# cocowy1/PPMStereo

Hardware: AMD Instinct MI355X
Metric: disparity-px/s (higher is better)
Workload: dtype bf16; 1 GPU; BASELINE config 2: T=5 clip at 320x512, iters=10, hot path only (3-scale cascade from encoder outputs: corr pyramid build + lookup, QAM pick, pick-and-play memory attention, ConvGRU3D update, heads, convex upsample, test_mode=True as PPMStereo.forward_batch_test calls it: predictions[-1] is the output, so the mask head, the convex upsampling and the full-resolution resize run only where their resu; T=5, H=320, W=512, iters=10, parallelism=replicas x1

## Files before the change

### include/ppms.h

```cpp
#ifndef PPMS_H
#define PPMS_H
#include <stdint.h>

#ifdef __cplusplus
extern "C" {
#endif

#define PPMS_OK 0
#define PPMS_EINVAL (-1)
#define PPMS_ELAUNCH (-2)
#define PPMS_ENODEV (-3)

#define PPMS_ABI_VERSION 4

int ppms_version(void);
const char* ppms_last_error(void);
int ppms_device_info(char* name, int name_cap, int* cu_count, int* clock_mhz);

int ppms_corr_build(const float* fmap1, const float* fmap2, float* const pyr[5], int B, int C, int H, int W, void* stream);

int ppms_corr_lookup(const float* const pyr[4], const float* flow, int flow_nhwc, float* out_nchw, void* out_hi, void* out_lo,
                     int out_ld, void* flow_sp_hi, void* flow_sp_lo, int flow_sp_ld, int B, int H, int W, void* stream);

typedef struct ppms_sp {
// ... 43 lines not shown
    ppms_epilogue epi[2];
} ppms_conv;

int ppms_conv_gemm2(const ppms_conv* desc, const ppms_conv* dev_desc, int wm_hint, void* stream);
int ppms_conv_gemm2_slices(const ppms_conv* desc);
int64_t ppms_conv_gemm2_slice_workspace_bytes(const ppms_conv* desc, int nslice);
int ppms_conv_gemm2_sliced(const ppms_conv* desc, const ppms_conv* dev_desc, int nslice, void* workspace, void* stream);
int ppms_conv_gemm2_ysweep_slices(const ppms_conv* desc);
int ppms_conv_gemm2_ysweep(const ppms_conv* desc, const ppms_conv* dev_desc, int nslice, void* workspace, void* stream);
int ppms_conv_gemm5_applicable(const ppms_conv* desc);
int ppms_conv_gemm5(const ppms_conv* desc, const ppms_conv* dev_desc, int nbt, void* stream);
int ppms_conv_gemm5_slices(const ppms_conv* desc);
int ppms_conv_gemm5_sliced(const ppms_conv* desc, const ppms_conv* dev_desc, int nbt, int nslice, void* workspace, void* stream);
int ppms_conv_gemm6_applicable(const ppms_conv* desc);
int ppms_conv_gemm6(const ppms_conv* desc, const ppms_conv* dev_desc, void* stream);
int ppms_gemm1_applicable(const ppms_conv* desc);
int ppms_gemm1(const ppms_conv* desc, const ppms_conv* dev_desc, int cb_hint, void* stream);
int ppms_conv_stream_applicable(const ppms_conv* desc);
int ppms_conv_stream(const ppms_conv* desc, const ppms_conv* dev_desc, int hint, void* stream);
int ppms_struct_sizes(int* sp, int* epilogue, int* conv);

int ppms_dwconv_gelu(ppms_sp x, ppms_sp y, const float* w, const float* b, int k, int BT, int H, int W, void* stream);
int ppms_flow_patch7(const float* flow_nhwc, ppms_sp patch, int BT, int H, int W, void* stream);
int ppms_unc_tail(ppms_sp x, const float* w, float bias, float* unc, float* partial, int BT, int HW, void* stream);

int ppms_nchw_to_sp(const float* src, ppms_sp dst, int BT, int C, int HW, void* stream);
int ppms_sp_to_nchw(ppms_sp src, float* dst, int BT, int C, int HW, void* stream);
int ppms_nchw_to_nhwc(const float* src, float* dst, int dst_ld, int BT, int C, int HW, void* stream);
int ppms_nhwc_to_nchw(const float* src, int src_ld, float* dst, int BT, int C, int HW, void* stream);
int ppms_f32_to_sp(const float* src, int src_ld, ppms_sp dst, int64_t pixels, void* stream);
// ... 103 lines not shown
```

### ppmstereo_amd/_lib.py

```python
from __future__ import annotations

import ctypes as C
import os
from typing import Optional

import torch

from . import build as _build

c_void_p, c_int, c_float, c_int64 = C.c_void_p, C.c_int, C.c_float, C.c_int64

EPI_STORE, EPI_RESID, EPI_RH, EPI_GRU, EPI_ADDF32 = range(5)
ATTN_P_BF16, ATTN_P_FP16 = 0, 1
ACT_NONE, ACT_RELU, ACT_GELU, ACT_SIGMOID, ACT_TANH, ACT_ELU1 = range(6)


def vt_image(v: torch.Tensor, p_format: int) -> torch.Tensor:
    b = v.to(torch.bfloat16)
    if p_format == ATTN_P_BF16:
        return b.contiguous()
    return b.float().clamp(-65504.0, 65504.0).to(torch.float16).contiguous().view(torch.bfloat16)


def vt_values(vt: torch.Tensor, p_format: int) -> torch.Tensor:
# ... 4 lines not shown
    _fields_ = [("hi", c_void_p), ("lo", c_void_p), ("ld", C.c_int32), ("c", C.c_int32)]


class Epilogue(C.Structure):
    _fields_ = [("kind", C.c_int32), ("act", C.c_int32), ("scale", c_float), ("n_valid", C.c_int32),
                ("out_sp", SP), ("out_f32", c_void_p), ("out_f32_ld", C.c_int32), ("vt_f16", C.c_int32), ("out_vt", c_void_p),
                ("aux_sp", SP), ("aux_f32", c_void_p), ("aux_f32_ld", C.c_int32), ("pre_f32_ld", C.c_int32),
                ("pre_f32", c_void_p)]


class Conv(C.Structure):
    _fields_ = [("seg", SP * 2), ("nseg", C.c_int32), ("groups", C.c_int32), ("w", c_void_p), ("bias", c_void_p),
                ("T", C.c_int32), ("H", C.c_int32), ("W", C.c_int32),
                ("kt", C.c_int32), ("kh", C.c_int32), ("kw", C.c_int32),
                ("M", C.c_int32), ("m_split", C.c_int32), ("t_halo", C.c_int32), ("lo_zero_from", C.c_int32), ("epi", Epilogue * 2)]


class ChainLayer(C.Structure):
    _fields_ = [("w", c_void_p), ("bias", c_void_p), ("post_s", c_void_p), ("post_t", c_void_p),
                ("M", C.c_int32), ("n_valid", C.c_int32), ("resid", C.c_int32)]


class ChainParams(C.Structure):
    _fields_ = [("inp", SP), ("out", SP), ("layer", ChainLayer * 3), ("nlayers", C.c_int32), ("P", C.c_int64)]


class YUVView(C.Structure):
    _fields_ = [("y", c_void_p), ("u", c_void_p), ("v", c_void_p), ("frame_stride_y", c_int64), ("frame_stride_c", c_int64),
                ("pitch_y", C.c_int32), ("pitch_c", C.c_int32), ("step_c", C.c_int32), ("reserved", C.c_int32)]

# ... 29 lines not shown
                                 c_int, c_int, c_int, c_int, c_void_p]),
    "ppms_conv_gemm2": (c_int, [C.POINTER(Conv), c_void_p, c_int, c_void_p]),
    "ppms_conv_gemm2_slices": (c_int, [C.POINTER(Conv)]),
    "ppms_conv_gemm2_slice_workspace_bytes": (C.c_int64, [C.POINTER(Conv), c_int]),
    "ppms_conv_gemm2_sliced": (c_int, [C.POINTER(Conv), c_void_p, c_int, c_void_p, c_void_p]),
    "ppms_conv_gemm2_ysweep_slices": (c_int, [C.POINTER(Conv)]),
    "ppms_conv_gemm2_ysweep": (c_int, [C.POINTER(Conv), c_void_p, c_int, c_void_p, c_void_p]),
    "ppms_gemm1_applicable": (c_int, [C.POINTER(Conv)]),
    "ppms_gemm1": (c_int, [C.POINTER(Conv), c_void_p, c_int, c_void_p]),
    "ppms_conv_stream_applicable": (c_int, [C.POINTER(Conv)]),
    "ppms_conv_stream": (c_int, [C.POINTER(Conv), c_void_p, c_int, c_void_p]),
    "ppms_conv_gemm5_applicable": (c_int, [C.POINTER(Conv)]),
    "ppms_conv_gemm5": (c_int, [C.POINTER(Conv), c_void_p, c_int, c_void_p]),
    "ppms_conv_gemm6_applicable": (c_int, [C.POINTER(Conv)]),
    "ppms_conv_gemm6": (c_int, [C.POINTER(Conv), c_void_p, c_void_p]),
    "ppms_conv_gemm5_slices": (c_int, [C.POINTER(Conv)]),
    "ppms_conv_gemm5_sliced": (c_int, [C.POINTER(Conv), c_void_p, c_int, c_int, c_void_p, c_void_p]),
    "ppms_struct_sizes": (c_int, [C.POINTER(c_int), C.POINTER(c_int), C.POINTER(c_int)]),
    "ppms_dwconv_gelu": (c_int, [SP, SP, c_void_p, c_void_p, c_int, c_int, c_int, c_int, c_void_p]),
    "ppms_flow_patch7": (c_int, [c_void_p, SP, c_int, c_int, c_int, c_void_p]),
    "ppms_unc_tail": (c_int, [SP, c_void_p, c_float, c_void_p, c_void_p, c_int, c_int, c_void_p]),
    "ppms_nchw_to_sp": (c_int, [c_void_p, SP, c_int, c_int, c_int, c_void_p]),
    "ppms_sp_to_nchw": (c_int, [SP, c_void_p, c_int, c_int, c_int, c_void_p]),
    "ppms_nchw_to_nhwc": (c_int, [c_void_p, c_void_p, c_int, c_int, c_int, c_int, c_void_p]),
    "ppms_nhwc_to_nchw": (c_int, [c_void_p, c_int, c_void_p, c_int, c_int, c_int, c_void_p]),
    "ppms_f32_to_sp": (c_int, [c_void_p, c_int, SP, c_int64, c_void_p]),
    "ppms_sp_to_f32": (c_int, [SP, c_void_p, c_int, c_int64, c_void_p]),
    "ppms_tap_gather_sum": (c_int, [c_void_p, c_int, c_void_p, c_void_p, c_int, c_void_p, c_int, c_int, c_int, c_int, c_int, c_int, c_int, c_int, c_int, c_void_p]),
    "ppms_flow_add": (c_int, [c_void_p, c_void_p, c_int, c_int64, c_void_p]),
    "ppms_convex_upsample": (c_int, [c_void_p, c_void_p, c_int, c_void_p, c_int, c_int, c_int, c_void_p]),
# ... 57 lines not shown
    try:
        path = _build.build(verbose=not os.path.exists(_build.LIB))
        lib = C.CDLL(path)
    except Exception as exc:
        raise RuntimeError(f"ppmstereo_amd: the HIP library libppms.so is missing and could not be built ({exc}); "
                           "there is no CPU fallback") from exc
    for name, (res, args) in _SIGS.items():
        fn = getattr(lib, name)
        fn.restype, fn.argtypes = res, args
    if lib.ppms_version() != 4:
        raise RuntimeError("ppmstereo_amd: libppms.so ABI version mismatch")
    a, b, c = c_int(), c_int(), c_int()
    lib.ppms_struct_sizes(C.byref(a), C.byref(b), C.byref(c))
    if (a.value, b.value, c.value) != (C.sizeof(SP), C.sizeof(Epilogue), C.sizeof(Conv)):
        raise RuntimeError("ppmstereo_amd: ctypes struct layout differs from include/ppms.h")
    lib.ppms_yuv_struct_sizes(C.byref(a), C.byref(b))
    if (a.value, b.value) != (C.sizeof(YUVView), C.sizeof(YUVMatrix)):
        raise RuntimeError("ppmstereo_amd: ctypes layout of ppms_yuv_view / ppms_yuv_matrix differs from include/ppms.h")
    lib.ppms_remap_struct_size(C.byref(a))
    if a.value != C.sizeof(RemapView):
        raise RuntimeError("ppmstereo_amd: ctypes layout of ppms_remap_view differs from include/ppms.h")
    if lib.ppms_egress_struct_size() != C.sizeof(Egress):
        raise RuntimeError("ppmstereo_amd: ctypes layout of ppms_egress differs from include/ppms.h")
    if lib.ppms_pwchain_param_bytes() != C.sizeof(ChainParams):
        raise RuntimeError("ppmstereo_amd: ChainParams layout differs from pwchain.hip")
    _lib = lib
    return lib


def check(rc: int) -> None:
# ... 48 lines not shown
```

### ppmstereo_amd/convplan.py

```python
from __future__ import annotations

import ctypes as C
from typing import Dict, Optional, Sequence

import torch

from . import _lib as L
from . import packing as _packing

CONV2 = 2
CONV5 = 5
GEMM1 = 6
STREAM = 7
CONV6 = 8
CONV2_SWEPT = "2s"
KERNEL_NAMES = {CONV2: "conv_gemm2", CONV5: "conv_gemm5", GEMM1: "gemm1", STREAM: "conv_stream", CONV6: "conv_gemm6"}
ALL_KERNELS = frozenset((CONV2, CONV2_SWEPT, CONV5, GEMM1, STREAM, CONV6))

TUNING = dict(
    conv6_grouped=True,
    attn_p="fp16",
)

KERNEL_TIMING = {"on": True}


def attn_p_format() -> int:
    fmt = TUNING["attn_p"]
    if fmt not in ("fp16", "bf16"):
        raise ValueError(f"TUNING['attn_p'] must be 'fp16' or 'bf16', got {fmt!r}")
    return L.ATTN_P_FP16 if fmt == "fp16" else L.ATTN_P_BF16


def _timed(fn, events):
    if events is not None and KERNEL_TIMING["on"]:
# ... 55 lines not shown
        if self.version not in (CONV5, CONV6) or lz <= 0 or lz >= cin or lz % (16 if self.version == CONV5 else 32):
            return 3.0
        if self.version == CONV6:
            nsweep = d.kh * d.kw if (d.kh > 1 or d.kw > 1) else 1
            if ((lz // 32) * nsweep) & 1:
                return 3.0
        return 3.0 - (cin - lz) / cin

    def __call__(self):
        _timed(self._launch, self.events)

    def _launch(self):
        L.check(self._fn(*self._args, L.stream_ptr()))


def epilogue(kind=L.EPI_STORE, act=L.ACT_NONE, scale=1.0, n_valid=0, out_sp: Optional[L.SP] = None, out_f32=None, out_f32_ld=0,
             out_vt=None, aux_sp: Optional[L.SP] = None, aux_f32=None, aux_f32_ld=0, pre_f32=None, pre_off=0, vt_f16=None) -> L.Epilogue:
    e = L.Epilogue()
    e.kind, e.act, e.scale, e.n_valid = kind, act, scale, n_valid
    if out_sp is not None:
        e.out_sp = out_sp
    e.out_f32 = None if out_f32 is None else out_f32.data_ptr()
    e.out_f32_ld = out_f32_ld
    e.out_vt = None if out_vt is None else out_vt.data_ptr()
    e.vt_f16 = attn_p_format() if vt_f16 is None else int(vt_f16)
    if aux_sp is not None:
        e.aux_sp = aux_sp
    e.aux_f32 = None if aux_f32 is None else aux_f32.data_ptr()
    e.aux_f32_ld = aux_f32_ld
    if pre_f32 is not None:
# ... 129 lines not shown
        d, k = _with_pack(desc, packs[CONV6], keep)
        if _fills_half(d) and lib.ppms_conv_gemm6_applicable(C.byref(d)) == 1:
            return ConvOp(d, k, CONV6, device=device)
    if CONV5 in packs:
        d, k = _with_pack(desc, packs[CONV5], keep)
        if _fills_half(d) and lib.ppms_conv_gemm5_applicable(C.byref(d)):
            return ConvOp(d, k, CONV5, device=device)
    if CONV2_SWEPT in packs and desc.kh > 1 and desc.kw == 1:
        d, k = _with_pack(desc, packs[CONV2_SWEPT], keep)
        if lib.ppms_conv_gemm2_ysweep_slices(C.byref(d)) > 0:
            return ConvOp(d, k, CONV2, ysweep=True, device=device)
    if CONV2 in packs:
        d, k = _with_pack(desc, packs[CONV2], keep)
        return ConvOp(d, k, CONV2, nslice=nslice, device=device)
    return None
```

### ppmstereo_amd/csrc/conv_gemm6.hip

```cpp
#include "common.h"
#include "conv_epilogue.h"
#include "conv_check.h"
#include <type_traits>

namespace {

constexpr int NT6 = 256;
constexpr int MAXP6 = 14;
__host__ __device__ constexpr int conv6_np(int cr) { return cr == 16 ? 14 : 9; }
constexpr int NBT6 = 13;
constexpr int STG6_ROWS = 7 * 16;
constexpr int EPI6_G = 2;


struct Geo6 {
    int tiles_x, tiles_y;
    int WH, WC;
    int hxl, hyl;
    int mode;
    int nsweep;
    int swx_n, inc, jump;
    int yinc, ywrap;
    int nchunk, n0;
    int cpw;
// ... 15 lines not shown
        g.dbg[(int64_t)blockIdx.x * 16 + (K)] = wall_clock64();                           \
        g.dbg[(int64_t)blockIdx.x * 16 + 8 + (K)] = (long long)__builtin_amdgcn_s_memtime(); \
    }
#else
#define CONV6_STAMP(K)
#endif

__device__ __forceinline__ void dma16_6(unsigned off, const u32x4& srd, unsigned lds_dst) {
    asm volatile("s_mov_b32 m0, %2\n\ts_nop 0\n\tbuffer_load_dwordx4 %0, %1, 0 offen lds" ::"v"(off), "s"(srd), "s"(lds_dst) : "memory");
}
constexpr unsigned CONV6_NUM_RECORDS = 0xFFFFFF00u;
constexpr unsigned CONV6_OOB = 0xFFFFFFF0u;

#include "conv6_asm.h"

template <int MB, int CR, bool STREAM = false, bool GRP = false, bool KS = false>
__global__ __launch_bounds__(NT6, 1) void conv6_kernel(const ppms_conv pv, const Geo6 g) {
    extern __shared__ __attribute__((aligned(16))) char smem[];
    const ppms_conv& p = pv;
    CONV6_STAMP(0)
    const int tid = threadIdx.x, lane = tid & 63;
    const int wave = __builtin_amdgcn_readfirstlane(tid >> 6);
    const int li = lane & 15, lkg = lane >> 4;
    constexpr bool DUAL = GRP || KS;
    const bool split = p.M == 128 && !KS;
    const int wm = (split || KS) ? (wave & 1) : wave;
    const int wn = split ? (wave >> 1) : 0;
    const int kg = KS ? (wave >> 1) : 0;
    const int nbw = split ? (wn ? 6 : 7) : NBT6;
    const int blk0 = wn ? 7 : 0;
    auto gchunk = [&](int grp, int c) { return c < g.lz0 ? grp * g.lz0 + c : g.lz0_full + grp * (g.nchunk - g.lz0) + (c - g.lz0); };
    auto wchunk = [&](int c) { return KS ? gchunk(kg, c) : c; };
// ... 307 lines not shown
        if (kg == 0) {
#pragma unroll
            for (int nl = 0; nl < 7; ++nl)
#pragma unroll
                for (int m = 0; m < 4; ++m) acc[m][nl] += *(const f32x4*)(xr + ((nl * 4 + m) * 64 + lane) * 4);
        } else {
#pragma unroll
            for (int nl = 0; nl < 6; ++nl)
#pragma unroll
                for (int m = 0; m < 4; ++m) acc[m][7 + nl] += *(const f32x4*)(xr + ((nl * 4 + m) * 64 + lane) * 4);
        }
        __syncthreads();
        e_nbw = kg ? 6 : 7;
        e_blk0 = kg ? 7 : 0;
    }

    constexpr int LD6 = 16 * MB + 4;
    float* stg = (float*)smem + wave * (STG6_ROWS * LD6);
    const int c_lo = wm * 16 * MB;
    const int q = lane & 7;
    const bool qok = q < 2 * MB;
    const int cout = c_lo + q * 8;
    const int lane_half = (cout >= p.m_split) ? 1 : 0;
    float b8[8];
    {
        const float* bp = p.bias + (qok ? cout : c_lo);
        const f32x4 b0 = gld<f32x4>(bp), b1 = gld<f32x4>(bp + 4);
#pragma unroll
        for (int j = 0; j < 4; ++j) {
            b8[j] = b0[j];
// ... 64 lines not shown
            using GL = std::integral_constant<int, EPI6_G>;
            const int cls = epilogue_class(e);
            if (cls == EPI_CLS_PLAIN) rows(I0{}, G2{});
            else if (cls == EPI_CLS_PRE) rows(I1{}, GL{});
            else if (cls == EPI_CLS_AUX) rows(I2{}, GL{});
            else if (cls == EPI_CLS_GRU) rows(I3{}, GL{});
            else if (cls == EPI_CLS_AUXPRE) rows(I5{}, GL{});
            else rows(I4{}, G1{});
        }
        }
    };
    using Z0 = std::integral_constant<int, 0>;
    if constexpr (KS) {
        if (kg == 0) do_pass(Z0{}, Z0{});
        else do_pass(Z0{}, std::integral_constant<int, 7>{});
    } else {
        do_pass(Z0{}, Z0{});
        do_pass(std::integral_constant<int, 1>{}, Z0{});
    }
    CONV6_STAMP(3)
}

static bool plan6(const ppms_conv* d, Geo6& g) {
    const bool grouped = d->groups == 2;
    if (grouped && !(d->nseg == 2 && d->seg[0].c == d->seg[1].c && d->M == 256 && d->m_split == 128 && d->kh == 1 && d->kw >= 3 && d->kw <= 5 && d->lo_zero_from == 0))
        return false;
    const bool stream = d->kw == 1 && d->kh == 1;
    g.mode = stream ? 4 : (d->kw > 1 && d->kh > 1) ? 2 : (d->kw > 1 ? 0 : 1);
    const int hx = (g.mode == 0 || g.mode == 2) ? d->kw - 1 : 0, hy = (g.mode == 1 || g.mode == 2) ? d->kh - 1 : 0;
    g.cpw = 32;
// ... 61 lines not shown
}

static bool serve6(const ppms_conv* d, Geo6& g) {
    CONV_REFUSE_IF((int64_t)d->T * d->H * d->W >= (1ll << 22), "conv_gemm6: volume %dx%dx%d too large for the packed window slots (< 2^22 pixels)", d->T, d->H, d->W);
    CONV_REFUSE_IF(!conv6_offsets_fit(d), "conv_gemm6: the lo plane of a segment must follow its hi plane inside one 4 GiB range (32-bit window offsets)");
    CONV_REFUSE_IF(!plan6(d, g), "conv_gemm6: not a convolution this kernel serves (a halo'd 16 x 13 window of <= 14 DMA pieces per thread; groups=%d: two equal "
                                 "segments, M = 256, m_split = 128, (1,1,3..5) taps)", d->groups);
    CONV_REFUSE_IF(conv6_lds(d, g) > 160 * 1024, "conv_gemm6: LDS budget exceeded (%zu B)", conv6_lds(d, g));
    return true;
}

template <int MB, int CR, bool STREAM = false, bool GRP = false, bool KS = false>
static void launch6(const ppms_conv* d, const Geo6& g, hipStream_t st) {
    static ppms_device_once once;
    once.run([] { (void)hipFuncSetAttribute((const void*)conv6_kernel<MB, CR, STREAM, GRP, KS>, hipFuncAttributeMaxDynamicSharedMemorySize, 160 * 1024); });
    hipLaunchKernelGGL((conv6_kernel<MB, CR, STREAM, GRP, KS>), dim3(g.tiles_x * g.tiles_y * d->T), dim3(NT6), conv6_lds(d, g), st, *d, g);
}

}

extern "C" int ppms_conv_gemm6_applicable(const ppms_conv* d) {
    Geo6 g;
    if (!conv_check_shape(RULES6, d) || !serve6(d, g)) return 0;
    const int64_t tiles = (int64_t)g.tiles_x * g.tiles_y * d->T;
    const int64_t cus = ppms_num_cus();
    if (tiles < cus * 25 / 32) return 0;
    const double fill = (double)g.P / ((double)((tiles + cus - 1) / cus) * cus * 16 * NBT6);
    return fill >= 0.85 ? 1 : 2;
}

#ifdef PPMS_CONV6_TIMING
extern "C" void ppms_debug_conv6_timing(long long* p) { g_conv6_dbg = p; }
#endif

extern "C" int ppms_conv_gemm6(const ppms_conv* d, const ppms_conv* dev_desc, void* stream) {
    Geo6 g;
    if (!conv_check_shape(RULES6, d) || !conv_check_operands(RULES6, d) || !serve6(d, g)) return PPMS_EINVAL;
    PPMS_REQUIRE(dev_desc != nullptr, "conv_gemm6: null device descriptor");
#ifdef PPMS_CONV6_TIMING
    g.dbg = g_conv6_dbg;
#endif
    hipStream_t st = (hipStream_t)stream;
    const bool grouped = d->groups == 2, plain = !grouped && !g.ks && g.mode != 4;
    if (plain && d->M != 192) {
// ... 2 lines not shown
        if (g.WH == 16) launch6<3, 16>(d, g, st); else if (g.WH == 18) launch6<3, 18>(d, g, st); else launch6<3, 20>(d, g, st);
    } else if (!grouped && !g.ks) {
        if (d->M != 192) launch6<4, 16, true>(d, g, st);
        else launch6<3, 16, true>(d, g, st);
    } else if (grouped) {
        launch6<4, 16, false, true>(d, g, st);
    } else if (g.WH == 16) {
        launch6<4, 16, false, false, true>(d, g, st);
    } else if (g.WH == 18) {
        launch6<4, 18, false, false, true>(d, g, st);
    } else {
        launch6<4, 20, false, false, true>(d, g, st);
    }
    return ppms_check_launch("conv_gemm6");
}
```

### ppmstereo_amd/engine.py

```python
from __future__ import annotations

import ctypes as C
import math
from typing import Dict, List, Optional

import torch

from . import _lib as L
from . import packing as _packing
from .convplan import (ALL_KERNELS, CONV2, CONV2_SWEPT, CONV6, KERNEL_TIMING, TUNING, ConvOp, PwChain, TimedCall,
                       attn_p_format, conv_desc, epilogue, pack_conv, plan_conv)

TOP_K = 5


def temporal_pe(T: int, channels: int) -> torch.Tensor:
    pos = torch.arange(T)
    pos = pos / pos[-1] * 1.0
    pos = pos.unsqueeze(1)
    div = 1.0 / (10000.0 ** (torch.arange(0, channels, 2).float() / channels))
    ang = pos * div
    pe = torch.zeros(T, channels)
    pe[:, 0::2] = torch.sin(ang)
    pe[:, 1::2] = torch.cos(ang)
    return pe

# ... 53 lines not shown
                    n_ = name[2:].replace("1_0", "1.0")
                    wt, bs = cat(gr + f"convz{n_}.weight", gr + f"convr{n_}.weight"), cat(gr + f"convz{n_}.bias", gr + f"convr{n_}.bias")
                else:
                    wt, bs = g(gr + f"convq{name[1:]}.weight"), g(gr + f"convq{name[1:]}.bias")
                w_h = torch.cat([wt[:, :128], wt[:, 256:]], 1).contiguous()
                put(name + "_i", wt[:, 128:256].contiguous(), bs, [128], kernels=ALL_KERNELS - {CONV2_SWEPT})
                put(name + "_h", w_h, None, [128, 256])
                beta = float(sd["aggregator.beta"].detach().double().reshape(-1)[0])
                wd = wt.double()
                w_x = torch.cat([wd[:, :128], wd[:, 256:384] + wd[:, 384:], beta * wd[:, 384:]], 1).float().contiguous()
                put(name + "_x", w_x, None, [128, 256])
        put("fh1", g("flow_head.conv1.weight"), g("flow_head.conv1.bias"), [128])
        w2 = g("flow_head.conv2.weight")
        put("fh2", w2.permute(2, 3, 4, 0, 1).reshape(54, 256, 1, 1, 1).contiguous(), None, [256])
        self.fh2_bias = g("flow_head.conv2.bias").contiguous()
        self.convex_3d = "mask_3d.0.weight" in sd
        mk = "mask_3d." if self.convex_3d else "mask_2d."
        put("m1", g(mk + "0.weight"), g(mk + "0.bias"), [128])
        put("m2", g(mk + "2.weight"), g(mk + "2.bias"), [256])
        self.mask_ch = 432 if self.convex_3d else 144
        self.beta = g("aggregator.beta").contiguous()
        self.attn = None
        if "time_attn.temporal_fc.weight" in sd:
            self.attn = {k: g(k) for k in sd if k.startswith("time_attn.") or k.startswith("space_attn.")}
            lin = lambda k: g(k)[:, :, None, None]
            ta, sa = "time_attn.", "space_attn.encoder_layer."
            w_fc, w_pj = g(ta + "temporal_fc.weight").double(), g(ta + "temporal_attn.proj.weight").double()
            w_ta = (w_fc @ w_pj).float().contiguous()
            b_ta = (w_fc @ g(ta + "temporal_attn.proj.bias").double() + g(ta + "temporal_fc.bias").double()).float().contiguous()
            put("ta_fc", w_ta[:, :, None, None], b_ta, [384])
# ... 148 lines not shown
        for tag, sfx, lz in ((("", "_h", 0), ("_x", "_x", 256)) if hoist else (("", "", 0),)):
            o["zr1_0" + tag] = self._conv("zr1_0" + sfx, [H[0].view(), x_all], (1, 1, 15), E(act=L.ACT_GELU, n_valid=128, out_sp=self.ZT.view(), **pre("zr1_0")),
                                          E(act=L.ACT_GELU, n_valid=128, out_sp=self.RT.view(), **pre("zr1_0", 128)), m_split=128, lo_zero_from=lz)
            o["q1" + tag] = self._conv("q1" + sfx, [self.RH.view(), x_all], (1, 1, 5),
                                       E(L.EPI_GRU, n_valid=128, out_sp=H[1].view(), aux_sp=H[0].view(), aux_f32=self.Z, aux_f32_ld=128, **pre("q1")), lo_zero_from=lz)
            for n, kk, src, dst in (("2", (1, 5, 1), 1, 2), ("3", (5, 1, 1), 2, 0)):
                o["zr" + n + tag] = self._conv("zr" + n + sfx, [H[src].view(), x_all], kk,
                                               E(act=L.ACT_SIGMOID, n_valid=128, out_f32=self.Z, out_f32_ld=128, **pre("zr" + n)),
                                               E(L.EPI_RH, n_valid=128, out_sp=self.RH.view(), aux_sp=H[src].view(), **pre("zr" + n, 128)), m_split=128,
                                               lo_zero_from=lz)
                o["q" + n + tag] = self._conv("q" + n + sfx, [self.RH.view(), x_all], kk,
                                              E(L.EPI_GRU, n_valid=128, out_sp=H[dst].view(), aux_sp=H[src].view(), aux_f32=self.Z, aux_f32_ld=128,
                                                **pre("q" + n)), lo_zero_from=lz)
        o["fh1"] = self._conv("fh1", [H[0].view()], (3, 3, 3), E(act=L.ACT_RELU, n_valid=256, out_sp=self.FH1.view()))
        o["fh2"] = self._conv("fh2", [self.FH1.view()], k1, E(n_valid=54, out_f32=self.FH2Y, out_f32_ld=64))
        o["m1"] = self._conv("m1", [H[0].view()], (3, 3, 3) if self.pk.convex_3d else k3, E(act=L.ACT_RELU, n_valid=256, out_sp=self.M1.view()))
        o["m2"] = self._conv("m2", [self.M1.view()], k1, E(scale=0.25, n_valid=self.pk.mask_ch, out_f32=self.MASK, out_f32_ld=self.pk.mask_ch))

    def _s(self):
        return L.stream_ptr()

    def load_nchw(self, x: torch.Tensor, dst: L.SP):
        x = x.contiguous().float()
        L.require_gpu(x)
        L.check(self.lib.ppms_nchw_to_sp(x.data_ptr(), dst, x.shape[0], x.shape[1], x.shape[2] * x.shape[3], self._s()))

    def store_nchw(self, src: L.SP, c: int) -> torch.Tensor:
        out = torch.empty(self.T, c, self.h, self.w, dtype=torch.float32, device=self.dev)
        L.check(self.lib.ppms_sp_to_nchw(src, out.data_ptr(), self.T, c, self.n, self._s()))
        return out
# ... 179 lines not shown
                                       self.pk.beta.data_ptr(), mf_in, self.X.view(256, 128), L.ptr(out_bf16), self.T, self.n,
                                       self.ATT_WS.data_ptr(), 0, self.attn_p, s))
        if self._health_on:
            L.check(self.lib.ppms_attn_redo_accumulate(self.ATT_WS.data_ptr(), self.T, self.ksel, self.n, 0, self._health.data_ptr(), s))
        self._x_hid = self.hid_mode
        if ev is not None:
            ev[1].record()
        if self.shard is not None and self.pk.attn is None:
            self._drain_xa_halo()
            self._xa_halo = self._halo_sp(self.XA, 2, async_op=True)

    def conv_ops(self, version: Optional[int] = None):
        return {k: v for k, v in self.op.items() if isinstance(v, ConvOp) and (version is None or v.version == version)}

    def conv_family_ops(self):
        fam = {k: v for k, v in self.op.items() if isinstance(v, (ConvOp, PwChain, TimedCall))}
        fam.update({f"to_qk_{i}": v for i, v in enumerate(self._qk_ops.values())})
        return fam

    def attn_redo_count(self):
        if self.n % 64:
            return 0, 0
        flags = self.ATT_WS.view(torch.int32)[self.T * self.ksel * self.n * 130:]
        g64 = (self.n + 255) // 256
        used = self.T * self.ksel * g64
        f = flags[:used * 2:2]
        torch.cuda.synchronize()
        return int(used), int((f != 0).sum().item())

    def enable_attn_health(self, on: bool = True):
        if on and self._health is None:
# ... 62 lines not shown
        if self.shard is not None:
            self._halo_sp(self.Hb[2], 2)
            if self._xa_halo is not None:
                self._xa_halo.wait()
                self._xa_halo = None
            else:
                self._halo_sp(self.XA, 2)
        o["zr3" + tag]()
        self._halo_sp(self.RH, 2)
        o["q3" + tag]()
        self._halo_sp(self.Hb[0], 1)
        if need_mask:
            with self._fork():
                o["m1"]()
                o["m2"]()
        o["fh1"]()
        o["fh2"]()
        self._halo_f32(self._FH2Y_full, 1)
        L.check(self.lib.ppms_tap_gather_sum(self.FH2Y.data_ptr(), 64, self.pk.fh2_bias.data_ptr(), self.DFLOW.data_ptr(), 4, self.FLOW.data_ptr(), 2,
                                             2, 3, 3, 3, self.T, self.h, self.w, self.halo, self._s()))
        if need_mask:
            self._join()

    def upsample(self) -> torch.Tensor:
        self.hbm["convex_upsample"]()
        return self.FLOW_OUT

    def egress(self, out: L.Egress, frame0: int, n_frames: int, pad_left: int, pad_top: int, h0: int, w0: int):
        if self.shard is not None:
            raise NotImplementedError("ScaleEngine.egress: a frame-sharded engine holds a part of the window")
        disparity_egress(self.FLOW_OUT, self.UNC.view(self.T, self.h, self.w), out, frame0, n_frames, pad_left, pad_top, h0, w0)

# ... 41 lines not shown
```

### ppmstereo_amd/packing.py

```python
from __future__ import annotations

from typing import List, Optional, Sequence, Tuple

import torch

BM, BK = 64, 32


def _pad_to(n: int, m: int) -> int:
    return (n + m - 1) // m * m


def split_bf16(x: torch.Tensor) -> Tuple[torch.Tensor, torch.Tensor]:
    hi = x.to(torch.bfloat16)
    lo = (x - hi.float()).to(torch.bfloat16)
    return hi, lo


def pack_conv2(weight: torch.Tensor, bias: Optional[torch.Tensor], seg_channels: Sequence[int],
               seg_padded: Optional[Sequence[int]] = None, cout_map: Optional[Sequence[int]] = None,
               m_pad: Optional[int] = None) -> Tuple[torch.Tensor, torch.Tensor, dict]:
    w = weight.detach().float()
    if w.dim() == 4:
        w = w[:, :, None]
# ... 104 lines not shown
def pack_conv6_grouped(weights: Sequence[torch.Tensor], biases: Sequence[Optional[torch.Tensor]], group_channels: int) -> Tuple[torch.Tensor, torch.Tensor, dict]:
    assert len(weights) == 2 and len(biases) == 2
    parts, bs, meta0 = [], [], None
    for w, b in zip(weights, biases):
        assert w.shape[0] <= 128 and w.shape[1] == group_channels, (tuple(w.shape), group_channels)
        packed, bias, meta = pack_conv6(w, b, [group_channels], None, None, 128)
        parts.append(packed.reshape(meta["nk"], 8, 2, 64, 8))
        bs.append(bias)
        assert meta0 is None or (meta0["nk"], meta0["taps"], meta0["cpad"]) == (meta["nk"], meta["taps"], meta["cpad"])
        meta0 = meta
    packed = torch.cat(parts, dim=1).contiguous()
    meta = dict(M=256, nk=meta0["nk"], taps=meta0["taps"], cpad=meta0["cpad"], seg_padded=[meta0["cpad"], meta0["cpad"]], version=8, groups=2)
    return packed.reshape(-1), torch.cat(bs), meta


def unpack_conv6_reference(packed: torch.Tensor, M: int, nk: int, taps, nchunk: int) -> torch.Tensor:
    kt, kh, kw = taps
    t = packed.reshape(nk, M // 16, 2, 64, 8).float()
    t = t[:, :, 0] + t[:, :, 1]
    t = t.reshape(kt * kh, nchunk, kw, M // 16, 4, 16, 8)
    t = t.permute(3, 5, 0, 2, 1, 4, 6)
    return t.reshape(M, kt * kh * kw * nchunk * 32)


def pack_gemm1(weight: torch.Tensor, bias: Optional[torch.Tensor], seg_channels: Sequence[int],
               seg_padded: Optional[Sequence[int]] = None, cout_map: Optional[Sequence[int]] = None,
               m_pad: Optional[int] = None) -> Tuple[torch.Tensor, torch.Tensor, dict]:
    w = weight.detach().float()
    w = w.reshape(w.shape[0], w.shape[1], -1)
    assert w.shape[2] == 1, "pack_gemm1: 1x1 kernels only"
# ... 96 lines not shown
```

Baseline: 23.26 million disparity-px/s.

## Fuse flow-head 1x1 conv into the conv6 3x3x3 producer epilogue

Adds a tail mode to the conv6 kernel. The ReLU'd fh1 accumulators are split into bf16 hi/lo in registers and multiplied by the packed fh2 1x1 weights with MFMA, with the cross-wave partial sums reduced through LDS before the fh2 epilogue stores. This removes the FH1 intermediate store and reload, plus one kernel launch, on every iteration. In exchange the producer kernel gets extra register pressure and LDS staging with syncthreads, and the path is limited to the plain M=256 layout with one epilogue half.

```diff
diff --git a/include/ppms.h b/include/ppms.h
--- a/include/ppms.h
+++ b/include/ppms.h
@@ -81,6 +81,20 @@
 int ppms_conv_gemm5_sliced(const ppms_conv* desc, const ppms_conv* dev_desc, int nbt, int nslice, void* workspace, void* stream);
 int ppms_conv_gemm6_applicable(const ppms_conv* desc);
 int ppms_conv_gemm6(const ppms_conv* desc, const ppms_conv* dev_desc, void* stream);
+typedef struct ppms_conv_tail {
+    const void* w;
+    const float* bias;
+    int32_t N;
+    int32_t n_valid;
+    int32_t src_half;
+    int32_t src_c0, src_c;
+    int32_t keep_src;
+    ppms_sp extra;
+    ppms_epilogue epi;
+} ppms_conv_tail;
+int ppms_conv_gemm6_tail_applicable(const ppms_conv* desc, const ppms_conv_tail* tail);
+int ppms_conv_gemm6_tail(const ppms_conv* desc, const ppms_conv* dev_desc, const ppms_conv_tail* tail, void* stream);
+int ppms_conv_tail_struct_size(void);
 int ppms_gemm1_applicable(const ppms_conv* desc);
 int ppms_gemm1(const ppms_conv* desc, const ppms_conv* dev_desc, int cb_hint, void* stream);
 int ppms_conv_stream_applicable(const ppms_conv* desc);
diff --git a/ppmstereo_amd/_lib.py b/ppmstereo_amd/_lib.py
--- a/ppmstereo_amd/_lib.py
+++ b/ppmstereo_amd/_lib.py
@@ -42,6 +42,11 @@
                 ("T", C.c_int32), ("H", C.c_int32), ("W", C.c_int32),
                 ("kt", C.c_int32), ("kh", C.c_int32), ("kw", C.c_int32),
                 ("M", C.c_int32), ("m_split", C.c_int32), ("t_halo", C.c_int32), ("lo_zero_from", C.c_int32), ("epi", Epilogue * 2)]
+
+
+class ConvTail(C.Structure):
+    _fields_ = [("w", c_void_p), ("bias", c_void_p), ("N", C.c_int32), ("n_valid", C.c_int32), ("src_half", C.c_int32),
+                ("src_c0", C.c_int32), ("src_c", C.c_int32), ("keep_src", C.c_int32), ("extra", SP), ("epi", Epilogue)]
 
 
 class ChainLayer(C.Structure):
@@ -101,6 +106,9 @@
     "ppms_conv_gemm5": (c_int, [C.POINTER(Conv), c_void_p, c_int, c_void_p]),
     "ppms_conv_gemm6_applicable": (c_int, [C.POINTER(Conv)]),
     "ppms_conv_gemm6": (c_int, [C.POINTER(Conv), c_void_p, c_void_p]),
+    "ppms_conv_gemm6_tail_applicable": (c_int, [C.POINTER(Conv), C.POINTER(ConvTail)]),
+    "ppms_conv_gemm6_tail": (c_int, [C.POINTER(Conv), c_void_p, C.POINTER(ConvTail), c_void_p]),
+    "ppms_conv_tail_struct_size": (c_int, []),
     "ppms_conv_gemm5_slices": (c_int, [C.POINTER(Conv)]),
     "ppms_conv_gemm5_sliced": (c_int, [C.POINTER(Conv), c_void_p, c_int, c_int, c_void_p, c_void_p]),
     "ppms_struct_sizes": (c_int, [C.POINTER(c_int), C.POINTER(c_int), C.POINTER(c_int)]),
@@ -188,6 +196,8 @@
     lib.ppms_struct_sizes(C.byref(a), C.byref(b), C.byref(c))
     if (a.value, b.value, c.value) != (C.sizeof(SP), C.sizeof(Epilogue), C.sizeof(Conv)):
         raise RuntimeError("ppmstereo_amd: ctypes struct layout differs from include/ppms.h")
+    if lib.ppms_conv_tail_struct_size() != C.sizeof(ConvTail):
+        raise RuntimeError("ppmstereo_amd: ctypes layout of ppms_conv_tail differs from include/ppms.h")
     lib.ppms_yuv_struct_sizes(C.byref(a), C.byref(b))
     if (a.value, b.value) != (C.sizeof(YUVView), C.sizeof(YUVMatrix)):
         raise RuntimeError("ppmstereo_amd: ctypes layout of ppms_yuv_view / ppms_yuv_matrix differs from include/ppms.h")
diff --git a/ppmstereo_amd/convplan.py b/ppmstereo_amd/convplan.py
--- a/ppmstereo_amd/convplan.py
+++ b/ppmstereo_amd/convplan.py
@@ -19,6 +19,7 @@
 
 TUNING = dict(
     conv6_grouped=True,
+    conv_tail=True,
     attn_p="fp16",
 )
 
@@ -104,6 +105,29 @@
         L.check(self._fn(*self._args, L.stream_ptr()))
 
 
+class ConvTailOp:
+
+    def __init__(self, desc: L.Conv, tail: L.ConvTail, keep: list, device=None):
+        self.desc, self.tail, self.version, self.nslice, self.wm_hint, self.ysweep = desc, tail, CONV6, 1, 0, False
+        device = torch.device("cuda", torch.cuda.current_device()) if device is None else torch.device(device)
+        self.dev = torch.frombuffer(bytearray(bytes(desc)), dtype=torch.uint8).clone().to(device)
+        self.keep, self.events = keep, None
+        self._fn, self._args = L.load().ppms_conv_gemm6_tail, (C.byref(desc), self.dev.data_ptr(), C.byref(tail))
+
+    def flops(self) -> float:
+        d = self.desc
+        return ConvOp.flops(self) + 2.0 * d.T * d.H * d.W * self.tail.n_valid * self.tail.src_c
+
+    def mfma_per_product(self) -> float:
+        return ConvOp.mfma_per_product(self)
+
+    def __call__(self):
+        _timed(self._launch, self.events)
+
+    def _launch(self):
+        L.check(self._fn(*self._args, L.stream_ptr()))
+
+
 def epilogue(kind=L.EPI_STORE, act=L.ACT_NONE, scale=1.0, n_valid=0, out_sp: Optional[L.SP] = None, out_f32=None, out_f32_ld=0,
              out_vt=None, aux_sp: Optional[L.SP] = None, aux_f32=None, aux_f32_ld=0, pre_f32=None, pre_off=0, vt_f16=None) -> L.Epilogue:
     e = L.Epilogue()
@@ -263,3 +287,18 @@
         d, k = _with_pack(desc, packs[CONV2], keep)
         return ConvOp(d, k, CONV2, nslice=nslice, device=device)
     return None
+
+
+def plan_conv_tail(producer: Optional[ConvOp], tail_pack: tuple, epi: L.Epilogue, src_half: int = 0, src_c0: int = 0, keep_src: bool = False,
+                   keep=(), device=None) -> Optional[ConvTailOp]:
+    if producer is None or producer.version != CONV6:
+        return None
+    packed, bias, meta = tail_pack
+    t = L.ConvTail()
+    t.w, t.bias, t.N, t.n_valid = packed.data_ptr(), bias.data_ptr(), meta["N"], epi.n_valid
+    t.src_half, t.src_c0, t.src_c, t.keep_src = src_half, src_c0, meta["src_c"], int(keep_src)
+    t.epi = epi
+    d = L.Conv.from_buffer_copy(bytes(producer.desc))
+    if L.load().ppms_conv_gemm6_tail_applicable(C.byref(d), C.byref(t)) != 1:
+        return None
+    return ConvTailOp(d, t, [packed, bias, *producer.keep, *keep], device=device)
diff --git a/ppmstereo_amd/csrc/conv_gemm6.hip b/ppmstereo_amd/csrc/conv_gemm6.hip
--- a/ppmstereo_amd/csrc/conv_gemm6.hip
+++ b/ppmstereo_amd/csrc/conv_gemm6.hip
@@ -53,8 +53,11 @@
 
 #include "conv6_asm.h"
 
-template <int MB, int CR, bool STREAM = false, bool GRP = false, bool KS = false>
-__global__ __launch_bounds__(NT6, 1) void conv6_kernel(const ppms_conv pv, const Geo6 g) {
+struct NoTail6 {};
+constexpr int TAIL6_LD = 68;
+constexpr int TAIL6_PB = 4;
+template <int MB, int CR, bool STREAM = false, bool GRP = false, bool KS = false, bool TAIL = false>
+__global__ __launch_bounds__(NT6, 1) void conv6_kernel(const ppms_conv pv, const Geo6 g, const std::conditional_t<TAIL, ppms_conv_tail, NoTail6> tl) {
     extern __shared__ __attribute__((aligned(16))) char smem[];
     const ppms_conv& p = pv;
     CONV6_STAMP(0)
@@ -392,6 +395,120 @@
         e_nbw = kg ? 6 : 7;
         e_blk0 = kg ? 7 : 0;
     }
+    if constexpr (TAIL) {
+        static_assert(MB == 4 && !STREAM && !DUAL, "the tail is written for the plain M = 256 layout");
+        float* const tst = (float*)smem;
+        const bool s_relu = p.epi[tl.src_half].act == PPMS_ACT_RELU;
+        const float s_scale = p.epi[tl.src_half].scale;
+        float pb[4][4];
+#pragma unroll
+        for (int m = 0; m < 4; ++m) {
+            const f32x4 b = gld<f32x4>(p.bias + wave * 64 + 16 * m + 4 * lkg);
+#pragma unroll
+            for (int j = 0; j < 4; ++j) pb[m][j] = b[j];
+        }
+        const ppms_epilogue te = tl.epi;
+        const bool t_plain = te.pre_f32 == nullptr;
+        const int tq = tid & 7;
+        auto tail_round = [&](const int tg) __attribute__((always_inline)) {
+            u32x4 tw[2][4][2];
+            const char* wb = (const char*)tl.w + (size_t)(tg * 4 + wave) * 16384 + lane * 16;
+#pragma unroll
+            for (int f = 0; f < 16; ++f) tw[f >> 3][(f >> 1) & 3][f & 1] = gld<u32x4>(wb + f * 1024);
+            float tb8[8];
+            {
+                const float* bp = tl.bias + tg * 64 + tq * 8;
+                const f32x4 b0 = gld<f32x4>(bp), b1 = gld<f32x4>(bp + 4);
+#pragma unroll
+                for (int j = 0; j < 4; ++j) tb8[j] = b0[j], tb8[4 + j] = b1[j];
+            }
+            auto tail_pass = [&](auto ps_tag) __attribute__((always_inline)) {
+                constexpr int ps = decltype(ps_tag)::value;
+#pragma unroll
+                for (int m = 0; m < 4; ++m)
+#pragma unroll
+                    for (int j = 0; j < 4; ++j) asm volatile("" : "+v"(pb[m][j]));
+#pragma unroll
+                for (int nl = 0; nl < TAIL6_PB; ++nl) {
+                    const int n = ps * TAIL6_PB + nl < NBT6 ? ps * TAIL6_PB + nl : NBT6 - 1;
+                    if (ps * TAIL6_PB + nl < NBT6) {
+                        bf16x8 bh[2], bl[2];
+#pragma unroll
+                        for (int m = 0; m < 4; ++m) {
+                            float y[4];
+#pragma unroll
+                            for (int j = 0; j < 4; ++j) {
+                                y[j] = acc[m][n][j] + pb[m][j];
+                                y[j] = ((s_relu && y[j] < 0.0f) ? 0.0f : y[j]) * s_scale;
+                            }
+#pragma unroll
+                            for (int j = 0; j < 4; ++j) {
+                                bf16_t hh, ll;
+                                split_bf16(y[j], hh, ll);
+                                bh[m >> 1][4 * (m & 1) + j] = hh;
+                                bl[m >> 1][4 * (m & 1) + j] = ll;
+                            }
+                        }
+#pragma unroll
+                        for (int nb = 0; nb < 4; ++nb) {
+                            f32x4 c = {0.0f, 0.0f, 0.0f, 0.0f};
+#pragma unroll
+                            for (int ks = 0; ks < 2; ++ks) {
+                                const bf16x8 wh = __builtin_bit_cast(bf16x8, tw[ks][nb][0]), wl = __builtin_bit_cast(bf16x8, tw[ks][nb][1]);
+                                c = __builtin_amdgcn_mfma_f32_16x16x32_bf16(wh, bh[ks], c, 0, 0, 0);
+                                c = __builtin_amdgcn_mfma_f32_16x16x32_bf16(wl, bh[ks], c, 0, 0, 0);
+                                c = __builtin_amdgcn_mfma_f32_16x16x32_bf16(wh, bl[ks], c, 0, 0, 0);
+                            }
+                            *(f32x4*)(tst + ((wave * TAIL6_PB + nl) * 16 + li) * TAIL6_LD + nb * 16 + 4 * lkg) = c;
+                        }
+                    }
+                }
+                __syncthreads();
+                constexpr int NPB = (ps + 1) * TAIL6_PB <= NBT6 ? TAIL6_PB : NBT6 - ps * TAIL6_PB;
+                auto trows = [&](auto cls_tag) __attribute__((always_inline)) {
+                    constexpr int CLS = decltype(cls_tag)::value;
+                    row8_aux aux[2];
+                    int64_t pixk[2];
+                    bool okk[2];
+#pragma unroll
+                    for (int k = 0; k < 2; ++k) {
+                        const int prow = (tid >> 3) + 32 * k;
+                        const int px = x0 + ps * TAIL6_PB + (prow >> 4), py = y0 + (prow & 15);
+                        okk[k] = prow < NPB * 16 && px < W && py < H;
+                        pixk[k] = (int64_t)(tf * H + py) * W + px;
+                        if (okk[k]) row8_fetch<CLS>(te, pixk[k], tg * 64 + tq * 8, aux[k]);
+                    }
+#pragma unroll
+                    for (int k = 0; k < 2; ++k) {
+                        const int prow = (tid >> 3) + 32 * k;
+                        float v[8];
+#pragma unroll
+                        for (int w4 = 0; w4 < 4; ++w4) {
+                            const float* sp = tst + (w4 * TAIL6_PB * 16 + prow) * TAIL6_LD + tq * 8;
+                            const f32x4 a = *(const f32x4*)sp, b = *(const f32x4*)(sp + 4);
+#pragma unroll
+                            for (int j = 0; j < 4; ++j) {
+                                v[j] = w4 ? v[j] + a[j] : a[j];
+                                v[4 + j] = w4 ? v[4 + j] + b[j] : b[j];
+                            }
+                        }
+#pragma unroll
+                        for (int j = 0; j < 8; ++j) v[j] += tb8[j];
+                        if (okk[k]) row8_finish<CLS>(te, v, pixk[k], tg * 64 + tq * 8, HW, aux[k]);
+                    }
+                };
+                if (t_plain) trows(std::integral_constant<int, EPI_CLS_PLAIN>{});
+                else trows(std::integral_constant<int, EPI_CLS_PRE>{});
+                __syncthreads();
+            };
+            static_assert((NBT6 + TAIL6_PB - 1) / TAIL6_PB == 4, "four passes below");
+            tail_pass(std::integral_constant<int, 0>{});
+            tail_pass(std::integral_constant<int, 1>{});
+            tail_pass(std::integral_constant<int, 2>{});
+            tail_pass(std::integral_constant<int, 3>{});
+        };
+        tail_round(0);
+    }
 
     constexpr int LD6 = 16 * MB + 4;
     float* stg = (float*)smem + wave * (STG6_ROWS * LD6);
@@ -486,6 +603,7 @@
     if constexpr (KS) {
         if (kg == 0) do_pass(Z0{}, Z0{});
         else do_pass(Z0{}, std::integral_constant<int, 7>{});
+    } else if constexpr (TAIL) {
     } else {
         do_pass(Z0{}, Z0{});
         do_pass(std::integral_constant<int, 1>{}, Z0{});
@@ -577,7 +695,50 @@
 static void launch6(const ppms_conv* d, const Geo6& g, hipStream_t st) {
     static ppms_device_once once;
     once.run([] { (void)hipFuncSetAttribute((const void*)conv6_kernel<MB, CR, STREAM, GRP, KS>, hipFuncAttributeMaxDynamicSharedMemorySize, 160 * 1024); });
-    hipLaunchKernelGGL((conv6_kernel<MB, CR, STREAM, GRP, KS>), dim3(g.tiles_x * g.tiles_y * d->T), dim3(NT6), conv6_lds(d, g), st, *d, g);
+    hipLaunchKernelGGL((conv6_kernel<MB, CR, STREAM, GRP, KS>), dim3(g.tiles_x * g.tiles_y * d->T), dim3(NT6), conv6_lds(d, g), st, *d, g, NoTail6{});
+}
+
+template <int CR>
+static void launch6_tail(const ppms_conv* d, const Geo6& g, const ppms_conv_tail* t, hipStream_t st) {
+    static ppms_device_once once;
+    once.run([] { (void)hipFuncSetAttribute((const void*)conv6_kernel<4, CR, false, false, false, true>, hipFuncAttributeMaxDynamicSharedMemorySize, 160 * 1024); });
+    hipLaunchKernelGGL((conv6_kernel<4, CR, false, false, false, true>), dim3(g.tiles_x * g.tiles_y * d->T), dim3(NT6), conv6_lds(d, g), st, *d, g, *t);
+}
+
+static bool serve6_tail(const ppms_conv* d, const Geo6& g, const ppms_conv_tail* t) {
+    CONV_REFUSE_IF(t == nullptr, "conv_gemm6_tail: null tail");
+    CONV_REFUSE_IF(t->N != 64, "conv_gemm6_tail: N=%d (64: one round of 64 tail couts; the ABI allows up to 128)", t->N);
+    CONV_REFUSE_IF(d->groups == 2 || g.ks || g.mode == 4 || d->M != 256,
+                   "conv_gemm6_tail: producer M=%d groups=%d taps (%d,%d,%d): the tail is served in the plain M = 256 layout only (spatial taps, one group)",
+                   d->M, d->groups, d->kt, d->kh, d->kw);
+    CONV_REFUSE_IF(g.WH != 18, "conv_gemm6_tail: producer kh=%d: the tail is built for windows of 18 rows (kh = 3: the 3x3 and 3x3x3 producers)", d->kh);
+    CONV_REFUSE_IF(t->src_half < 0 || t->src_half >= conv_halves(d), "conv_gemm6_tail: src_half=%d (the producer has %d)", t->src_half, conv_halves(d));
+    const int h_rows = t->src_half ? d->M - d->m_split : (d->m_split < d->M ? d->m_split : d->M);
+    CONV_REFUSE_IF(t->src_c0 < 0 || t->src_c <= 0 || t->src_c0 + t->src_c > h_rows,
+                   "conv_gemm6_tail: src_c0=%d src_c=%d: the input range must lie inside epilogue half %d (%d rows)", t->src_c0, t->src_c, t->src_half, h_rows);
+    CONV_REFUSE_IF(conv_halves(d) != 1 || t->keep_src != 0,
+                   "conv_gemm6_tail: keep_src=%d, %d epilogue halves: served for a producer of ONE half that is not stored (keep_src = 0)", t->keep_src, conv_halves(d));
+    CONV_REFUSE_IF(t->extra.hi != nullptr || t->extra.lo != nullptr || t->extra.c != 0, "conv_gemm6_tail: extra (c=%d): extra input channels are not served", t->extra.c);
+    const ppms_epilogue& se = d->epi[t->src_half];
+    CONV_REFUSE_IF(se.kind != PPMS_EPI_STORE || se.pre_f32 != nullptr || se.out_vt != nullptr,
+                   "conv_gemm6_tail: epi[%d] of the producer (kind=%d) must be a STORE epilogue without pre_f32 / out_vt", t->src_half, se.kind);
+    CONV_REFUSE_IF(se.act != PPMS_ACT_NONE && se.act != PPMS_ACT_RELU, "conv_gemm6_tail: epi[%d].act=%d of the producer (NONE or RELU)", t->src_half, se.act);
+    CONV_REFUSE_IF(t->epi.out_vt != nullptr, "conv_gemm6_tail: tail epi.out_vt is not served");
+    CONV_REFUSE_IF(t->epi.kind != PPMS_EPI_STORE, "conv_gemm6_tail: tail epi.kind=%d: a STORE epilogue only", t->epi.kind);
+    CONV_REFUSE_IF(conv6_lds(d, g) < (size_t)4 * TAIL6_PB * 16 * TAIL6_LD * 4, "conv_gemm6_tail: the launch's LDS (%zu B) does not hold the tail's staging area", conv6_lds(d, g));
+    return true;
+}
+
+static bool tail6_operands(const ppms_conv_tail* t) {
+    const ppms_epilogue& e = t->epi;
+    CONV_REFUSE_IF(t->w == nullptr || t->bias == nullptr || !conv_al16(t->w) || !conv_al16(t->bias), "conv_gemm6_tail: w/bias missing or not 16-byte aligned (w=%p bias=%p)", t->w, (const void*)t->bias);
+    CONV_REFUSE_IF(e.n_valid <= 0 || e.n_valid > t->N || e.n_valid != t->n_valid, "conv_gemm6_tail: n_valid=%d epi.n_valid=%d (equal, 1..N=%d)", t->n_valid, e.n_valid, t->N);
+    CONV_REFUSE_IF(e.pre_f32 != nullptr && e.n_valid % 4, "conv_gemm6_tail: tail epi.n_valid=%d must be a multiple of 4 with pre_f32", e.n_valid);
+    const char* why = epilogue_row8_check(e);
+    CONV_REFUSE_IF(why != nullptr, "conv_gemm6_tail: tail epi: %s", why);
+    CONV_REFUSE_IF(e.out_sp.hi != nullptr && e.out_sp.lo == nullptr, "conv_gemm6_tail: tail epi.out_sp has no lo plane");
+    CONV_REFUSE_IF(e.out_sp.hi == nullptr && e.out_f32 == nullptr, "conv_gemm6_tail: tail epi has no output (out_sp / out_f32)");
+    return true;
 }
 
 }
@@ -591,6 +752,14 @@
     const double fill = (double)g.P / ((double)((tiles + cus - 1) / cus) * cus * 16 * NBT6);
     return fill >= 0.85 ? 1 : 2;
 }
+
+extern "C" int ppms_conv_gemm6_tail_applicable(const ppms_conv* d, const ppms_conv_tail* t) {
+    Geo6 g;
+    if (!conv_check_shape(RULES6, d) || !serve6(d, g) || !serve6_tail(d, g, t)) return 0;
+    return ppms_conv_gemm6_applicable(d);
+}
+
+extern "C" int ppms_conv_tail_struct_size(void) { return (int)sizeof(ppms_conv_tail); }
 
 #ifdef PPMS_CONV6_TIMING
 extern "C" void ppms_debug_conv6_timing(long long* p) { g_conv6_dbg = p; }
@@ -623,3 +792,15 @@
     }
     return ppms_check_launch("conv_gemm6");
 }
+
+extern "C" int ppms_conv_gemm6_tail(const ppms_conv* d, const ppms_conv* dev_desc, const ppms_conv_tail* t, void* stream) {
+    Geo6 g;
+    if (!conv_check_shape(RULES6, d) || !conv_check_operands(RULES6, d) || !serve6(d, g) || !serve6_tail(d, g, t) || !tail6_operands(t)) return PPMS_EINVAL;
+    PPMS_REQUIRE(dev_desc != nullptr, "conv_gemm6_tail: null device descriptor");
+#ifdef PPMS_CONV6_TIMING
+    g.dbg = g_conv6_dbg;
+#endif
+    hipStream_t st = (hipStream_t)stream;
+    launch6_tail<18>(d, g, t, st);
+    return ppms_check_launch("conv_gemm6_tail");
+}
diff --git a/ppmstereo_amd/engine.py b/ppmstereo_amd/engine.py
--- a/ppmstereo_amd/engine.py
+++ b/ppmstereo_amd/engine.py
@@ -8,8 +8,8 @@
 
 from . import _lib as L
 from . import packing as _packing
-from .convplan import (ALL_KERNELS, CONV2, CONV2_SWEPT, CONV6, KERNEL_TIMING, TUNING, ConvOp, PwChain, TimedCall,
-                       attn_p_format, conv_desc, epilogue, pack_conv, plan_conv)
+from .convplan import (ALL_KERNELS, CONV2, CONV2_SWEPT, CONV6, KERNEL_TIMING, TUNING, ConvOp, ConvTailOp, PwChain, TimedCall,
+                       attn_p_format, conv_desc, epilogue, pack_conv, plan_conv, plan_conv_tail)
 
 TOP_K = 5
 
@@ -93,6 +93,7 @@
         w2 = g("flow_head.conv2.weight")
         put("fh2", w2.permute(2, 3, 4, 0, 1).reshape(54, 256, 1, 1, 1).contiguous(), None, [256])
         self.fh2_bias = g("flow_head.conv2.bias").contiguous()
+        self.tails = {"fh12": _packing.pack_tail(w2.permute(2, 3, 4, 0, 1).reshape(54, 256), None, 0, mb=4)}
         self.convex_3d = "mask_3d.0.weight" in sd
         mk = "mask_3d." if self.convex_3d else "mask_2d."
         put("m1", g(mk + "0.weight"), g(mk + "0.bias"), [128])
@@ -271,6 +272,10 @@
                                                 **pre("q" + n)), lo_zero_from=lz)
         o["fh1"] = self._conv("fh1", [H[0].view()], (3, 3, 3), E(act=L.ACT_RELU, n_valid=256, out_sp=self.FH1.view()))
         o["fh2"] = self._conv("fh2", [self.FH1.view()], k1, E(n_valid=54, out_f32=self.FH2Y, out_f32_ld=64))
+        if TUNING["conv_tail"] and "fh12" in self.pk.tails:
+            op = plan_conv_tail(o["fh1"], self.pk.tails["fh12"], o["fh2"].desc.epi[0], keep=[self.FH2Y], device=self.dev)
+            if op is not None:
+                o["fh12"] = op
         o["m1"] = self._conv("m1", [H[0].view()], (3, 3, 3) if self.pk.convex_3d else k3, E(act=L.ACT_RELU, n_valid=256, out_sp=self.M1.view()))
         o["m2"] = self._conv("m2", [self.M1.view()], k1, E(scale=0.25, n_valid=self.pk.mask_ch, out_f32=self.MASK, out_f32_ld=self.pk.mask_ch))
 
@@ -480,7 +485,7 @@
         return {k: v for k, v in self.op.items() if isinstance(v, ConvOp) and (version is None or v.version == version)}
 
     def conv_family_ops(self):
-        fam = {k: v for k, v in self.op.items() if isinstance(v, (ConvOp, PwChain, TimedCall))}
+        fam = {k: v for k, v in self.op.items() if isinstance(v, (ConvOp, ConvTailOp, PwChain, TimedCall))}
         fam.update({f"to_qk_{i}": v for i, v in enumerate(self._qk_ops.values())})
         return fam
 
@@ -573,8 +578,11 @@
             with self._fork():
                 o["m1"]()
                 o["m2"]()
-        o["fh1"]()
-        o["fh2"]()
+        if "fh12" in o:
+            o["fh12"]()
+        else:
+            o["fh1"]()
+            o["fh2"]()
         self._halo_f32(self._FH2Y_full, 1)
         L.check(self.lib.ppms_tap_gather_sum(self.FH2Y.data_ptr(), 64, self.pk.fh2_bias.data_ptr(), self.DFLOW.data_ptr(), 4, self.FLOW.data_ptr(), 2,
                                              2, 3, 3, 3, self.T, self.h, self.w, self.halo, self._s()))
diff --git a/ppmstereo_amd/packing.py b/ppmstereo_amd/packing.py
--- a/ppmstereo_amd/packing.py
+++ b/ppmstereo_amd/packing.py
@@ -142,6 +142,39 @@
     return packed.reshape(-1), torch.cat(bs), meta
 
 
+def tail_wave_couts(mb: int) -> torch.Tensor:
+    wave, step, kg, j = torch.meshgrid(torch.arange(4), torch.arange(2), torch.arange(4), torch.arange(8), indexing="ij")
+    blk = 2 * step + (j >> 2)
+    cout = 16 * mb * wave + 16 * blk + 4 * kg + (j & 3)
+    return torch.where(blk < mb, cout, torch.full_like(cout, -1))
+
+
+def pack_tail(weight: torch.Tensor, bias: Optional[torch.Tensor], src_c0: int, mb: int = 4, half_base: int = 0,
+              n_pad: Optional[int] = None) -> Tuple[torch.Tensor, torch.Tensor, dict]:
+    w = weight.detach().float()
+    w = w.reshape(w.shape[0], w.shape[1], -1)
+    assert w.shape[2] == 1, "pack_tail: 1x1 kernels only"
+    w = w[:, :, 0]
+    n, c = w.shape
+    N = _pad_to(n, 64) if n_pad is None else n_pad
+    assert N % 64 == 0 and N >= n and mb in (3, 4)
+    cout = tail_wave_couts(mb).to(w.device)
+    ci = cout - half_base - src_c0
+    ok = (cout >= 0) & (ci >= 0) & (ci < c)
+    full = torch.zeros(N, c + 1, dtype=torch.float32, device=w.device)
+    full[:n, :c] = w
+    t = full[:, torch.where(ok, ci, torch.full_like(ci, c))]
+    t = t.reshape(N // 64, 4, 16, 4, 2, 4, 8).permute(0, 3, 4, 1, 5, 2, 6).contiguous()
+    t = t.reshape(N // 64, 4, 2, 4, 64, 8)
+    hi, lo = split_bf16(t)
+    packed = torch.stack([hi, lo], dim=4).contiguous()
+    b = torch.zeros(N, dtype=torch.float32, device=w.device)
+    if bias is not None:
+        b[:n] = bias.detach().float()
+    meta = dict(N=N, n=n, src_c0=src_c0, src_c=c, mb=mb, half_base=half_base)
+    return packed.reshape(-1), b, meta
+
+
 def unpack_conv6_reference(packed: torch.Tensor, M: int, nk: int, taps, nchunk: int) -> torch.Tensor:
     kt, kh, kw = taps
     t = packed.reshape(nk, M // 16, 2, 64, 8).float()
```

New measurement: 23.44 million disparity-px/s, median of 6. About the same (+0.8%).
